# xiph/vorbis

Hardware: AMD Instinct MI355X
Metric: audio blocks/s (2048-sample MDCT+psy) @1/2/4/8 GPU; % HBM roofline (higher is better)
Workload: dtype f32

## Files before the change

include/vorbis_amd.h:

```cpp
#ifndef VORBIS_AMD_H
#define VORBIS_AMD_H

#include <stddef.h>
#include <stdint.h>
#include "vamd_setup.h"

#ifdef __cplusplus
extern "C" {
#endif

#define VAMD_OK        0
#define VAMD_EFAULT   (-129)
#define VAMD_EIMPL    (-130)
#define VAMD_EINVAL   (-131)
#define VAMD_EVERSION (-134)
#define VAMD_EDOMAIN    (-140)
#define VAMD_ENONFINITE (-141)

#define VAMD_BLOCKTYPE_IMPULSE    0
#define VAMD_BLOCKTYPE_PADDING    1
#define VAMD_BLOCKTYPE_TRANSITION 0
#define VAMD_BLOCKTYPE_LONG       1

#define VAMD_POSTS_STRIDE 32
// ... 5 lines not shown
#define vamd_create(ctx, setup_blob, blob_bytes, device) \
  vamd_create_abi((ctx), (setup_blob), (blob_bytes), (device), VAMD_ABI_VERSION)

void vamd_destroy(vamd_ctx *ctx);

const char *vamd_last_error(const vamd_ctx *ctx);

int vamd_set_stream(vamd_ctx *ctx, void *hip_stream);

int vamd_reserve(vamd_ctx *ctx, int W, long max_blocks);

int vamd_profile(vamd_ctx *ctx, int enable);
int vamd_stage_ms(vamd_ctx *ctx, float *ms, int nstages, int *runs);

int vamd_debug_cycles(vamd_ctx *ctx, int enable, unsigned long long *out80);

int vamd_clock_probe(vamd_ctx *ctx, unsigned long long *acc3);

int vamd_calib_copy(vamd_ctx *ctx, void *dst, const void *src, size_t bytes);

int vamd_channels(const vamd_ctx *ctx);
int vamd_blocksize(const vamd_ctx *ctx, int W);
int vamd_posts(const vamd_ctx *ctx, int W);


int vamd_mdct_forward_batch(vamd_ctx *ctx, int W, const float *in, float *out, long nframes);

typedef struct vamd_batch_desc {
  int         W;
  long        nblocks;
// ... 263 lines not shown
```

vorbis_amd/api.py:

```python
import ctypes as C
import os
import struct

import numpy as np

_HERE = os.path.dirname(os.path.abspath(__file__))

VAMD_OK, VAMD_EFAULT, VAMD_EIMPL, VAMD_EINVAL, VAMD_EVERSION, VAMD_EDOMAIN, VAMD_ENONFINITE = 0, -129, -130, -131, -134, -140, -141
ABI_VERSION = 9
QUANT_LIMIT_SQUARE, QUANT_LIMIT_INT = 46340, 0x7fffff80
STATUS_RANGE, STATUS_NONFINITE = 1, 2
LEVEL_TRANSFORM, LEVEL_PSY, LEVEL_FULL = 1, 2, 3
POSTS_STRIDE = 32
BLOCKTYPE_IMPULSE, BLOCKTYPE_PADDING, BLOCKTYPE_TRANSITION, BLOCKTYPE_LONG = 0, 1, 0, 1

EXPORTED_SYMBOLS = ["vamd_create_abi", "vamd_encode_blocks", "vamd_clock_probe", "vamd_quant_limit", "vamd_config_string", "vamd_destroy", "vamd_last_error", "vamd_set_stream", "vamd_reserve",
                    "vamd_channels", "vamd_blocksize", "vamd_posts", "vamd_mdct_forward_batch",
                    "vamd_analyze_batch", "vamd_analyze_stream", "vamd_analyze_block", "vamd_profile",
                    "vamd_stage_ms", "vamd_debug_cycles", "vamd_analyze_stream_mixed", "vamd_envelope_search_batch",
                    "vamd_envelope_search", "vamd_envelope_geometry", "vamd_residue_capacity", "vamd_analyze_block_res", "vamd_analyze_batch_managed", "vamd_analyze_block_managed",
                    "vamd_packet_capacity", "vamd_encode_block", "vamd_submaps", "vamd_residue_offset", "vamd_analyze_streams_mixed",
                    "vamd_plan_streams", "vamd_gather_blocks", "vamd_plan_fetch",
                    "vamd_batcher_create", "vamd_batcher_destroy", "vamd_batcher_attach", "vamd_batcher_detach",
                    "vamd_batcher_encode_block", "vamd_batcher_last_error", "vamd_batcher_stats", "vamd_batcher_context", "vamd_batcher_report",
                    "vamd_input_status", "vamd_calib_copy", "vamd_abi_version", "vamd_plan_streams_whole", "vamd_plan_streams_whole_v", "vamd_feed_wrote_v", "vamd_device_count", "vamd_batcher_create_multi",
                    "vamd_feed_create", "vamd_feed_destroy", "vamd_feed_lanes", "vamd_feed_device", "vamd_feed_buffer", "vamd_feed_wrote",
                    "vamd_feed_packets", "vamd_feed_release", "vamd_feed_last_error", "vamd_feed_create_live", "vamd_feed_wrote_live",
                    "vamd_analyze_streams_mixed_managed", "vamd_bitrate_init_states", "vamd_bitrate_walk",
                    "vamd_feed_ogg_headers", "vamd_feed_ogg_serials", "vamd_feed_ogg", "vamd_feed_ogg_headers_live",
                    "vamd_feed_ogg_comments", "vamd_feed_ogg_flush",
                    "vamd_feed_buffer_on", "vamd_feed_wrote_device", "vamd_feed_wrote_live_device", "vamd_feed_source_done",
                    "vamd_analyze_batch_synth", "vamd_synth_streams", "vamd_synth_check", "vamd_feed_decoded"]
PACKETBLOBS = 15

# ... 124 lines not shown
    L.vamd_destroy.restype = None
    L.vamd_last_error.argtypes = [_vp]
    L.vamd_last_error.restype = C.c_char_p
    L.vamd_set_stream.argtypes = [_vp, _vp]
    L.vamd_input_status.argtypes = [_vp, C.POINTER(C.c_long), C.POINTER(C.c_long)]
    L.vamd_reserve.argtypes = [_vp, C.c_int, C.c_long]
    L.vamd_channels.argtypes = [_vp]
    L.vamd_blocksize.argtypes = [_vp, C.c_int]
    L.vamd_posts.argtypes = [_vp, C.c_int]
    L.vamd_mdct_forward_batch.argtypes = [_vp, C.c_int, _vp, _vp, C.c_long]
    L.vamd_analyze_batch.argtypes = [_vp, C.POINTER(_Desc), C.POINTER(_IO), C.c_int]
    L.vamd_analyze_stream.argtypes = [_vp, C.POINTER(_Desc), C.POINTER(_IO), C.POINTER(C.c_float)]
    L.vamd_analyze_block.argtypes = [_vp, C.POINTER(_vp), C.c_int, C.c_int, C.c_int, C.c_int, C.c_float, _vp, _vp,
                                     _vp, _vp, _vp, _vp, C.POINTER(C.c_float)]
    L.vamd_debug_cycles.argtypes = [_vp, C.c_int, _vp]
    L.vamd_calib_copy.argtypes = [_vp, _vp, _vp, C.c_size_t]
    L.vamd_analyze_stream_mixed.argtypes = [_vp, C.POINTER(_Desc), C.POINTER(_IO), C.POINTER(_Desc), C.POINTER(_IO), _vp,
                                            C.c_long, C.POINTER(C.c_float)]
    L.vamd_analyze_streams_mixed.argtypes = [_vp, C.POINTER(_Desc), C.POINTER(_IO), C.POINTER(_Desc), C.POINTER(_IO), _vp, _vp,
                                             C.c_long, C.c_long, _vp]
    L.vamd_envelope_search_batch.argtypes = [_vp, _vp, C.c_long, C.c_long, C.c_long, C.c_long, _vp, _vp]
    L.vamd_envelope_search.argtypes = [_vp, C.POINTER(_vp), C.c_long, _vp, _vp]
    L.vamd_envelope_geometry.argtypes = [_vp, C.POINTER(C.c_int), C.POINTER(C.c_int)]
    L.vamd_residue_capacity.argtypes = [_vp, C.c_int]
    L.vamd_analyze_block_res.argtypes = [_vp, C.POINTER(_vp), C.c_int, C.c_int, C.c_int, C.c_int, C.c_float] + [_vp] * 10
    L.vamd_analyze_batch_managed.argtypes = [_vp, C.POINTER(_Desc), C.POINTER(_IO), C.POINTER(_MIO)]
    L.vamd_analyze_batch_synth.argtypes = [_vp, C.POINTER(_Desc), C.POINTER(_IO), _vp]
    L.vamd_synth_check.argtypes = [_vp, C.c_int]
    L.vamd_synth_streams.argtypes = [_vp, C.POINTER(_Plan), C.c_long, C.c_long, _vp, _vp, _vp, _vp, _vp]
    L.vamd_analyze_block_managed.argtypes = [_vp, C.POINTER(_vp), C.c_int, C.c_int, C.c_int, C.c_int, C.c_float] + [_vp] * 9
# ... 122 lines not shown
        runs = C.c_int(0)
        self._check(self.L.vamd_stage_ms(self.h, ms, 8, C.byref(runs)))
        return dict(zip(self.STAGES, [float(x) for x in ms])), runs.value

    def clock_probe(self, acc):
        if acc is not None:
            self._need_tensor(acc, self.torch.int64, "acc", numel=3)
        self._clk = acc
        self._check(self.L.vamd_clock_probe(self.h, _vp(acc.data_ptr()) if acc is not None else None))

    def debug_cycles(self, enable=True, read=False):
        out = np.zeros(80, dtype=np.uint64)
        self._check(self.L.vamd_debug_cycles(self.h, 1 if enable else 0, _vp(out.ctypes.data) if read else None))
        return out.reshape(5, 16)

    def calib_copy(self, dst, src):
        nbytes = src.numel() * src.element_size()
        assert dst.numel() * dst.element_size() == nbytes
        self._check(self.L.vamd_calib_copy(self.h, _vp(dst.data_ptr()), _vp(src.data_ptr()), nbytes))

    def reserve(self, W, max_blocks):
        self._check(self.L.vamd_reserve(self.h, W, max_blocks))

    def input_status(self):
        a, b = C.c_long(0), C.c_long(0)
        r = self.L.vamd_input_status(self.h, C.byref(a), C.byref(b))
        if r not in (VAMD_OK, VAMD_EDOMAIN, VAMD_ENONFINITE):
            self._check(r)
        self.last_input_code = r
        return int(a.value), int(b.value)
# ... 1076 lines not shown
```

vorbis_amd/csrc/k_tone.h:

```cpp
#pragma once
#include "vamd_wave.h"
#include "vamd_params.h"

namespace vamd {

#define VAMD_NEGINF (-9999.f)
#define VAMD_LINES_PAD(nl) (((nl) + 31) & ~31)

VAMD_HOSTDEV int seed_pad_lo(int linesper) { return (VAMD_EHMER_OFFSET * linesper + (linesper >> 1) + 3) & ~3; }
VAMD_HOSTDEV int seed_pad_hi(int linesper) { return ((VAMD_EHMER_MAX - VAMD_EHMER_OFFSET) * linesper + 3) & ~3; }
template <int LP = 0>
VAMD_DEV void seed_curve_scatter(float *seed, const float *__restrict__ band_rows ,
                                 int stride, float amp, int oc, int linesper_rt, float dBoffset, bool active) {
  const int linesper = LP ? LP : linesper_rt;
  int choice = (int)(((double)(amp + dBoffset) - 30.) * (double).1f);
  choice = choice < 0 ? 0 : choice;
  choice = choice > VAMD_P_LEVELS - 1 ? VAMD_P_LEVELS - 1 : choice;
  const F4 *__restrict__ row = (const F4 *)(band_rows + choice * stride);
  float *p = seed + (oc - VAMD_EHMER_OFFSET * linesper - (linesper >> 1));
  int p0 = VAMD_EHMER_MAX, p1 = 0;
  if (active) {
    const F2 posts = *(const F2 *)((const float *)row + VAMD_EHMER_MAX);
    p0 = (int)posts.x;
    p1 = (int)posts.y;
// ... 18 lines not shown
#define VAMD_TF_RUN_LINES 8
#endif
#ifndef VAMD_TF_GROUP_FOLD
#define VAMD_TF_GROUP_FOLD 0
#endif
#if VAMD_GPU
VAMD_DEV float tone_min(float a, float b) { return __builtin_amdgcn_fmed3f(a, b, VAMD_NEGINF); }
#define VAMD_TF_RUN_LOOP _Pragma("unroll 1")
#else
VAMD_DEV float tone_min(float a, float b) { return b < a ? b : a; }
#define VAMD_TF_RUN_LOOP
#endif
#include "k_tone_fold.inc"

#define VAMD_RING 16
VAMD_DEV int tone_chase_thread(const float *__restrict__ seeds, int linesper, int n, float *ring_amp, int *ring_pos,
                               int rstride, int rlane, unsigned short *__restrict__ surv) {
  int stack = 0, hmax = 0;
  unsigned long long wlo = 0, whi = 0;
  int nw = 0;
  auto emit = [&](int pos) {
    wlo = (wlo >> 16) | (whi << 48);
    whi = (whi >> 16) | ((unsigned long long)(unsigned)pos << 48);
    nw++;
    if ((nw & 7) == 0) {
      unsigned long long *dst = (unsigned long long *)(surv + nw - 8);
      dst[0] = wlo;
      dst[1] = whi;
    }
  };
  float a1 = 0.f, a2 = 0.f;
  int p1 = 0, p2 = 0;
  const F4 *q = (const F4 *)seeds;
  const int nblk = (n + 31) >> 5;
  F4 w[8];
#pragma unroll
  for (int k = 0; k < 8; k++) w[k] = q[k];
  for (int b = 0; b < nblk; b++) {
    float blk[32];
#pragma unroll
    for (int k = 0; k < 8; k++) blk[4 * k] = w[k].x, blk[4 * k + 1] = w[k].y, blk[4 * k + 2] = w[k].z, blk[4 * k + 3] = w[k].w;
    if (b + 1 < nblk) {
#pragma unroll
      for (int k = 0; k < 8; k++) w[k] = q[8 * b + 8 + k];
    }
#pragma unroll
    for (int j = 0; j < 32; j++) {
      const int i = (b << 5) + j;
      if (i < n) {
        const float s = blk[j];
        if (stack >= 2) {
          while (!(s < a1) && i < p1 + linesper && a1 <= a2 && i < p2 + linesper) {
            stack--;
            a1 = a2;
            p1 = p2;
            if (stack < 2) break;
            const int slot = (stack - 2) & (VAMD_RING - 1);
            a2 = ring_amp[slot * rstride + rlane];
            p2 = ring_pos[slot * rstride + rlane];
          }
        }
        const int slot = stack & (VAMD_RING - 1);
        if (stack == hmax) {
          if (stack >= VAMD_RING) emit(ring_pos[slot * rstride + rlane]);
          hmax++;
        }
        ring_amp[slot * rstride + rlane] = s;
        ring_pos[slot * rstride + rlane] = i;
        stack++;
        a2 = a1;
        p2 = p1;
        a1 = s;
        p1 = i;
      }
    }
  }
  for (int k = hmax > VAMD_RING ? hmax - VAMD_RING : 0; k < stack; k++) emit(ring_pos[(k & (VAMD_RING - 1)) * rstride + rlane]);
  for (int k = nw & ~7; k < nw; k++) {
    const int sh = 16 * (8 - (nw & 7) + (k & 7));
    surv[k] = (unsigned short)(sh < 64 ? wlo >> sh : whi >> (sh - 64));
  }
  return stack;
}

struct ChaseChunk {
  uint32_t popped;
  uint32_t sig_in;
  uint32_t sig_out;
  int exact;
};
VAMD_DEV ChaseChunk chase_chunk(const float *seeds, int linesper, int n, int s, int e, int warm, uint32_t enter,
                                float *ring_amp, int *ring_pos, int rstride, int rlane) {
  ChaseChunk out;
  out.popped = out.sig_in = out.sig_out = 0;
  const int ws = warm < 0 ? s : (s - warm > 0 ? s - warm : 0);
  out.exact = ws == 0;
  const int stop = e + linesper - 1 < n ? e + linesper - 1 : n;
  int stack = 0;
  float a1 = 0.f, a2 = 0.f;
  int p1 = 0, p2 = 0;
  if (warm < 0 && s > 0) {
    auto push = [&](float a, int pos) {
      const int slot = stack & (VAMD_RING - 1);
      ring_amp[slot * rstride + rlane] = a;
      ring_pos[slot * rstride + rlane] = pos;
      stack++;
      a2 = a1;
      p2 = p1;
      a1 = a;
      p1 = pos;
    };
    push(0.f, -(1 << 24));
    const int lo = s - linesper + 1;
    for (int k = 0; k < linesper - 1; k++)
      if (lo + k >= 0 && ((enter >> k) & 1u)) push(seeds[lo + k], lo + k);
  }
  auto window = [&](int t) {
    uint32_t m = 0;
    const int lo = t - linesper + 1;
    for (int k = stack - 1; k >= 0 && k >= stack - linesper; k--) {
      const int pos = k == stack - 1 ? p1 : (k == stack - 2 ? p2 : ring_pos[(k & (VAMD_RING - 1)) * rstride + rlane]);
      if (pos < lo) break;
      m |= 1u << (pos - lo);
    }
    return m;
  };
  for (int i = ws; i < stop; i++) {
    if (i == s) out.sig_in = window(s);
    if (i == e) out.sig_out = window(e);
    const float sv = seeds[i];
    if (stack >= 2) {
      while (!(sv < a1) && i < p1 + linesper && a1 <= a2 && i < p2 + linesper) {
        if (p1 >= s && p1 < e) out.popped |= 1u << (p1 - s);
        stack--;
        a1 = a2;
        p1 = p2;
        if (stack < 2) break;
        const int slot = (stack - 2) & (VAMD_RING - 1);
        a2 = ring_amp[slot * rstride + rlane];
        p2 = ring_pos[slot * rstride + rlane];
      }
    }
    const int slot = stack & (VAMD_RING - 1);
    ring_amp[slot * rstride + rlane] = sv;
    ring_pos[slot * rstride + rlane] = i;
    stack++;
    a2 = a1;
    p2 = p1;
    a1 = sv;
    p1 = i;
  }
  return out;
}

template <int LP>
VAMD_DEV ChaseChunk chase_chunk_regs(const float *seeds, int n, int s, int e, int cs, int warm, uint32_t enter) {
  constexpr int WN = LP - 1;
  constexpr uint32_t WMASK = (1u << WN) - 1u;
  ChaseChunk out;
  out.popped = out.sig_in = out.sig_out = 0;
  const int ws = warm < 0 ? s : s - warm;
  out.exact = ws <= 0;
  const int stop = e + LP - 1 < n ? e + LP - 1 : n;
  const int steps = (warm < 0 ? 0 : warm) + cs + LP - 1;
  uint32_t m = 0;
  float st[WN];
#pragma unroll
// ... 177 lines not shown
```

vorbis_amd/csrc/vamd_batch.h:

```cpp
#pragma once
struct WsPlan {
  float *mdct_raw, *logmdct, *logfft, *noise, *tone, *mdct, *local, *ampin, *ampglob, *seed;
  float *peaks;
  unsigned short *surv;
  int32_t *nsurv;
  ilog_t *ilogmask;
  int32_t *iwork, *posts, *post_valid, *nonzero;
  int32_t *wrapped;
  unsigned char *status;
};

static int run_peaks_stride(const PsyP &P) { return (P.nruns + 3) & ~3; }

static int plan(vamd_ctx *c, int W, long nb, const vamd_batch_io *io, int level, WsPlan *p) {
  const size_t ch = c->B.channels, n2 = c->B.bs[W] / 2;
  const size_t per = (size_t)nb * ch * n2 * 4;
  p->wrapped = nullptr;
  void *v;
#define PICK(field, user, slot, bytes)                     \
  do {                                                     \
    if (user) {                                            \
      p->field = user;                                     \
    } else {                                               \
      int r__ = ws_get(c, W, vamd_ctx::slot, (bytes), &v); \
// ... 26 lines not shown
    PICK(iwork, io ? io->iwork : nullptr, WS_IWORK, per);
    PICK(posts, io ? io->posts : nullptr, WS_POSTS, (size_t)nb * ch * VAMD_POSTS_STRIDE * 4);
    PICK(post_valid, io ? io->post_valid : nullptr, WS_POSTVALID, (size_t)nb * ch * 4);
    PICK(nonzero, io ? io->nonzero : nullptr, WS_NONZERO, (size_t)nb * ch * 4);
    if (io && io->packets) PICK(wrapped, (int32_t *)nullptr, WS_WRAPPED, (size_t)nb * ch * VAMD_POSTS_STRIDE * 4);
  }
#undef PICK
  return VAMD_OK;
}

int vamd_reserve(vamd_ctx *c, int W, long max_blocks) {
  DeviceGuard dev_guard(c);
  if (!c || (W != 0 && W != 1) || max_blocks < 1) return VAMD_EINVAL;
  WsPlan p;
  return plan(c, W, max_blocks, nullptr, VAMD_LEVEL_FULL, &p);
}

#define VAMD_SWITCH_LOGN(logn)   \
  switch (logn) {                \
    case 8: VAMD_GO(8); break;   \
    case 9: VAMD_GO(9); break;   \
    case 10: VAMD_GO(10); break; \
    case 11: VAMD_GO(11); break; \
    case 12: VAMD_GO(12); break; \
    default: VAMD_GO(0);         \
  }
#define VAMD_SWITCH_BINS(n2)                                                                \
  switch (n2) {                                                                             \
    case 32: VAMD_GO(5); break;                                                             \
    case 64: VAMD_GO(6); break;                                                             \
// ... 272 lines not shown
  return ((size_t)(nlp + (P0.ngroups > P1.ngroups ? P0.ngroups : P1.ngroups) + 1) * 4 + 15) & ~(size_t)15;
}
static bool fold_in_floor(const vamd_ctx *c, const BatchRun *R, int level) {
  const bool fold_env = !c->K.fold_separate;
  return fold_env && level >= VAMD_LEVEL_FULL && !R->M && c->B.xf[R->W].n / 2 <= 64 * 4 * VAMD_QPL;
}

static long noise_teams_per_cu(const vamd_ctx *c, int n2, size_t lds, bool overlap, bool alone, bool fold_later) {
  const int nw = n2 >= 256 ? 4 : (n2 >= 64 ? n2 / 64 : 1);
  long per_cu = (long)(c->lds_per_block / lds);
  if (per_cu > 32 / nw) per_cu = 32 / nw;
  const int noise_cap = c->K.noise_teams;
  if (noise_cap > 0) {
    if (per_cu > noise_cap) per_cu = noise_cap;
  } else if (overlap) {
    const int beside = c->K.noise_waves > 0 ? c->K.noise_waves : (alone ? 20 : 24);
    const long cap = (fold_later ? beside : 16) / nw;
    if (per_cu > cap) per_cu = cap > 0 ? cap : 1;
  }
  return per_cu < 1 ? 1 : per_cu;
}

static void launch_masks(vamd_ctx *c, BatchRun *R, int level, bool forked, bool alone) {
  if (R->nb == 0 || level < VAMD_LEVEL_PSY) return;
  const int W = R->W, ch = c->B.channels;
  const WsPlan &p = R->p;
  const DescP &d = R->d;
  const PsyP &P0 = c->B.psy[2 * W], &P1 = c->B.psy[2 * W + 1];
  const int n2 = c->B.xf[W].n / 2, nl = P0.total_octave_lines;
  const unsigned gcb = (unsigned)(R->nb * ch);
  hipStream_t s = c->stream;
  const bool overlap = masks_overlap(c, R);
  const bool fold_later = fold_in_floor(c, R, level);
  if (overlap && !forked) {
    (void)hipEventRecord(c->ev_fork, c->stream);
    (void)hipStreamWaitEvent(c->side, c->ev_fork, 0);
  }
  const int nlp = VAMD_LINES_PAD(nl);
  const size_t seed_lds = (size_t)(seed_pad_lo(P0.eighth_octave_lines) + nlp + seed_pad_hi(P0.eighth_octave_lines)) * 4;
  const long wave_max_cb = c->K.chase_wave_max;
  const bool by_wave = (long)gcb <= wave_max_cb && P0.eighth_octave_lines <= 16 && nl <= 2048;
  const bool lp8 = P0.eighth_octave_lines == 8 && P1.eighth_octave_lines == 8;
  const bool merge_env = !c->K.masks_separate;
  const bool merged = merge_env && !overlap && by_wave && lp8;
  if (merged) {
    const size_t nlds = (size_t)5 * VAMD_NZ_STRIDE(n2) * 4, tlds = seed_lds + (size_t)VAMD_RING * 8;
#define VAMD_GO(L)                                                                                                          \
  hipLaunchKernelGGL((k_noise_tone<L, 8>), dim3(2 * gcb), dim3(64 * NoiseGeom<L>::NW), nlds > tlds ? nlds : tlds, s, P0, P1, d, ch, \
                     (long)gcb, p.mdct_raw, p.noise, nlp, run_peaks_stride(P0), p.peaks, p.local, p.ampglob,                  \
                     R->make_ampmax ? p.ampglob : nullptr, p.seed, p.surv, p.nsurv)
    VAMD_SWITCH_BINS(n2)
#undef VAMD_GO
    prof_mark(c, VAMD_ST_NOISE);
  } else {
    const size_t lds = (size_t)5 * VAMD_NZ_STRIDE(n2) * 4;
    const long per_cu = noise_teams_per_cu(c, n2, lds, overlap, alone, fold_later);
    const unsigned grid = (unsigned)((long)gcb < per_cu * c->num_cus ? (long)gcb : per_cu * c->num_cus);
#define VAMD_GO(L)                                                                                                    \
  hipLaunchKernelGGL(k_noise<L>, dim3(grid), dim3(64 * NoiseGeom<L>::NW), lds, s, P0, P1, d, ch, (long)gcb, p.mdct_raw, \
                     p.noise)
    VAMD_SWITCH_BINS(n2)
#undef VAMD_GO
    prof_mark(c, VAMD_ST_NOISE);
  }
  if (overlap) s = c->side;
  {
    if (merged) {
    } else if (by_wave && lp8) {
      hipLaunchKernelGGL(k_tone_seed_chase<8>, dim3(gcb), dim3(64), seed_lds + (size_t)VAMD_RING * 8, s, P0, P1, d, ch, nlp,
                         run_peaks_stride(P0), p.peaks, p.local, p.ampglob, R->make_ampmax ? p.ampglob : nullptr, p.seed, p.surv,
                         p.nsurv);
    } else {
      if (lp8)
        hipLaunchKernelGGL(k_tone_seed<8>, dim3(gcb), dim3(64), seed_lds, s, P0, P1, d, ch, nlp, run_peaks_stride(P0), p.peaks, p.local,
                           p.ampglob, R->make_ampmax ? p.ampglob : nullptr, p.seed);
      else
        hipLaunchKernelGGL(k_tone_seed<0>, dim3(gcb), dim3(64), seed_lds, s, P0, P1, d, ch, nlp, run_peaks_stride(P0), p.peaks, p.local,
                           p.ampglob, R->make_ampmax ? p.ampglob : nullptr, p.seed);
      if (by_wave)
        hipLaunchKernelGGL(k_tone_chase_wave, dim3(gcb), dim3(64), (size_t)nlp * 4 + (size_t)VAMD_RING * 64 * 8, s,
                           P0.eighth_octave_lines, nl, nlp, d, p.seed, p.surv, p.nsurv);
      else
        hipLaunchKernelGGL(k_tone_chase, dim3((gcb + VAMD_CHASE_LANES - 1) / VAMD_CHASE_LANES), dim3(VAMD_CHASE_LANES),
                           (size_t)VAMD_RING * VAMD_CHASE_LANES * 8, s,
                           P0.eighth_octave_lines, nl, nlp, (long)gcb, d, p.seed, p.surv, p.nsurv);
    }
    if (!fold_later)
      hipLaunchKernelGGL(k_tone_fold, dim3(gcb), dim3(64), fold_lds_bytes(nlp, P0, P1), s, P0, P1, d, ch, nlp, p.seed, p.surv,
                         p.nsurv, p.local, p.tone);
  }
  if (overlap) (void)hipEventRecord(join_event(c, R), c->side);
}

static void launch_floor_on(vamd_ctx *c, BatchRun *R, int level) {
  if (R->nb == 0) return;
  const ResBufs &rb = R->rb;
  const int W = R->W, ch = c->B.channels;
  const WsPlan &p = R->p;
  const DescP &d = R->d;
  const vamd_managed_io *M = R->M;
// ... 351 lines not shown
```

vorbis_amd/csrc/vamd_kernels.h:

```cpp
#pragma once
extern __shared__ __attribute__((aligned(16))) unsigned char vamd_smem[];

__device__ __forceinline__ int d_lW(const DescP &d, long b) { return d.lW ? d.lW[b] : d.u_lW; }
__device__ __forceinline__ int d_nW(const DescP &d, long b) { return d.nW ? d.nW[b] : d.u_nW; }
__device__ __forceinline__ int d_bt(const DescP &d, long b) { return d.blocktype ? d.blocktype[b] : d.u_blocktype; }
__device__ __forceinline__ float d_amp(const DescP &d, long b) { return d.ampmax_in ? d.ampmax_in[b] : d.u_ampmax_in; }
__device__ __forceinline__ void flag_range(const DescP &d, long i) {
  const unsigned char old = d.status[i];
  if (!(old & VAMD_STATUS_RANGE)) {
    d.status[i] = old | VAMD_STATUS_RANGE;
    if (!old) atomicAdd(d.bad, 1u);
  }
}

#define VAMD_XF_WAVES 8
#ifndef VAMD_FLOOR_PAIR_MIN_LONG
#define VAMD_FLOOR_PAIR_MIN_LONG 0x7fffffffL
#endif
#ifndef VAMD_FLOOR_PAIR_MIN_SHORT
#define VAMD_FLOOR_PAIR_MIN_SHORT 16384L
#endif

struct XformLds {
  XformP P;
// ... 394 lines not shown
  const PsyP &P = d_bt(d, blk) ? P1 : P0;
  float g_amp;
  if (ampmax_make) {
    g_amp = d_amp(d, blk);
    for (int c = 0; c < ch; c++) {
      const float l = local_ampmax[blk * ch + c];
      if (l > g_amp) g_amp = l;
    }
    if (LANE == 0 && cb == blk * ch) ampmax_make[blk] = g_amp;
  } else {
    g_amp = ampmax_glob[blk];
  }
  const int nl = P.total_octave_lines;
  float *seed = (float *)vamd_smem + seed_pad_lo(LP);
  float *ring_amp = seed + nlp + seed_pad_hi(LP);
  int *ring_pos = (int *)(ring_amp + VAMD_RING);
  PhaseClock pc;
  pc.start(d.dbg ? d.dbg + 32 : nullptr);
  tone_seed_block<LP>(P, peaks + cb * nrp, g_amp, local_ampmax[cb], seed, pc);
  WAVE_FOR(i, nlp) {
    if (i >= nl) seed[i] = VAMD_NEGINF;
    seed_g[cb * nlp + i] = seed[i];
  }
  WAVE_SYNC();
  const int cs = (nl + 63) / 64;
  const int s0 = LANE * cs < nl ? LANE * cs : nl, e0 = s0 + cs < nl ? s0 + cs : nl;
  unsigned short *out = surv + cb * nlp;
  bool accepted = false;
  ChaseChunk r;
  r.popped = r.sig_in = r.sig_out = 0;
  r.exact = 1;
// ... 15 lines not shown
        const ChaseChunk t = chase_chunk_regs<LP>(seed, nl, s0, e0, cs, -1, prev_out);
        used = prev_out;
        r.popped = t.popped;
        r.sig_out = t.sig_out;
      }
    }
  }
  if (accepted) {
    const uint32_t alive = ~r.popped & (e0 - s0 >= 32 ? ~0u : ((1u << (e0 - s0)) - 1u));
    const int cnt = __builtin_popcount(alive);
    const int incl = wave_scan_sum(cnt);
    int at = incl - cnt;
    for (uint32_t m = alive; m; m &= m - 1) out[at++] = (unsigned short)(s0 + __builtin_ctz(m));
    if (LANE == 63) nsurv[cb] = incl;
  } else if (LANE == 0) {
    nsurv[cb] = tone_chase_thread(seed, LP, nl, ring_amp, ring_pos, 1, 0, out);
  }
  pc.mark(2);
  pc.flush();
}
template <int LP>
__global__ __launch_bounds__(64) void k_tone_seed_chase(PsyP P0, PsyP P1, DescP d, int ch, int nlp, int nrp,
                                                        const float *__restrict__ peaks,
                                                        const float *__restrict__ local_ampmax,
                                                        const float *__restrict__ ampmax_glob, float *__restrict__ ampmax_make,
                                                        float *__restrict__ seed_g, unsigned short *__restrict__ surv,
                                                        int *__restrict__ nsurv) {
  tone_seed_chase_run<LP>(P0, P1, d, ch, nlp, nrp, peaks, local_ampmax, ampmax_glob, ampmax_make, seed_g, surv, nsurv, blockIdx.x);
}

template <int LOGN2, int LP>
// ... 1 lines not shown
                                                                          const float *__restrict__ mdct_raw, float *__restrict__ noise,
                                                                          int nlp, int nrp, const float *__restrict__ peaks,
                                                                          const float *__restrict__ local_ampmax,
                                                                          const float *__restrict__ ampmax_glob, float *__restrict__ ampmax_make,
                                                                          float *__restrict__ seed_g, unsigned short *__restrict__ surv,
                                                                          int *__restrict__ nsurv) {
  if ((long)blockIdx.x < ncb) {
    noise_teams_once<LOGN2>(P0, P1, d, ch, mdct_raw, noise);
  } else if (threadIdx.x < 64) {
    tone_seed_chase_run<LP>(P0, P1, d, ch, nlp, nrp, peaks, local_ampmax, ampmax_glob, ampmax_make, seed_g, surv, nsurv,
                            (long)blockIdx.x - ncb);
  }
}

#define VAMD_CHASE_LANES 64
__global__ __launch_bounds__(64) void k_tone_chase(int linesper, int nl, int nlp, long ncb, DescP d,
                                                   const float *__restrict__ seed_g,
                                                   unsigned short *__restrict__ surv, int *__restrict__ nsurv) {
  float *ring_amp = (float *)vamd_smem;
  int *ring_pos = (int *)(ring_amp + VAMD_RING * VAMD_CHASE_LANES);
  const long cb = (long)blockIdx.x * VAMD_CHASE_LANES + threadIdx.x;
  PhaseClock pc;
  pc.start(d.dbg ? d.dbg + 32 : nullptr);
  const bool probe = d.clk && blockIdx.x == 0 && threadIdx.x == 0;
  unsigned long long w0 = 0;
  long long t0 = 0;
  if (probe) w0 = wall_clock64(), t0 = clock64();
  if (cb < ncb)
    nsurv[cb] = tone_chase_thread(seed_g + cb * nlp, linesper, nl, ring_amp, ring_pos, VAMD_CHASE_LANES, threadIdx.x, surv + cb * nlp);
  if (probe) {
    atomicAdd(d.clk, (unsigned long long)(clock64() - t0));
    atomicAdd(d.clk + 1, wall_clock64() - w0);
    atomicAdd(d.clk + 2, 1ull);
  }
  pc.mark(2);
  pc.flush();
}

__global__ __launch_bounds__(64) void k_tone_chase_wave(int linesper, int nl, int nlp, DescP d,
                                                        const float *__restrict__ seed_g,
                                                        unsigned short *__restrict__ surv, int *__restrict__ nsurv) {
  float *seed = (float *)vamd_smem;
  float *ring_amp = seed + nlp;
  int *ring_pos = (int *)(ring_amp + VAMD_RING * 64);
  const long cb = blockIdx.x;
  WAVE_FOR(q, nlp >> 2)((F4 *)seed)[q] = ((const F4 *)(seed_g + cb * nlp))[q];
  WAVE_SYNC();
  const int cs = (nl + 63) / 64;
  const int s0 = LANE * cs < nl ? LANE * cs : nl, e0 = s0 + cs < nl ? s0 + cs : nl;
  unsigned short *out = surv + cb * nlp;
  bool accepted = false;
  ChaseChunk r;
  r.popped = r.sig_in = r.sig_out = 0;
  r.exact = 1;
  unsigned long long fm = __ballot(s0 < nl && chase_flat_chunk(seed, s0, e0));
  int longest = 0;
  for (; fm && longest <= VAMD_CHASE_FLAT_MAX; longest++) fm &= fm << 1;
  if (longest <= VAMD_CHASE_FLAT_MAX) {
    if (s0 < nl) r = chase_chunk(seed, linesper, nl, s0, e0, VAMD_CHASE_WARM * linesper, 0, ring_amp, ring_pos, 64, LANE);
    uint32_t used = r.sig_in;
    for (int rd = 0; rd <= VAMD_CHASE_ROUNDS; rd++) {
      const uint32_t prev_out = (uint32_t)wave_shift_up1((int)r.sig_out, 0);
      const bool need = s0 < nl && !r.exact && used != prev_out;
      if (!__any(need)) {
        accepted = true;
        break;
      }
      if (rd == VAMD_CHASE_ROUNDS) break;
      if (need) {
        const ChaseChunk t = chase_chunk(seed, linesper, nl, s0, e0, -1, prev_out, ring_amp, ring_pos, 64, LANE);
        used = prev_out;
        r.popped = t.popped;
        r.sig_out = t.sig_out;
      }
    }
  }
  if (accepted) {
    const uint32_t alive = ~r.popped & (e0 - s0 >= 32 ? ~0u : ((1u << (e0 - s0)) - 1u));
    const int cnt = __builtin_popcount(alive);
    const int incl = wave_scan_sum(cnt);
    int at = incl - cnt;
    for (uint32_t m = alive; m; m &= m - 1) out[at++] = (unsigned short)(s0 + __builtin_ctz(m));
    if (LANE == 63) nsurv[cb] = incl;
  } else if (LANE == 0) {
    nsurv[cb] = tone_chase_thread(seed, linesper, nl, ring_amp, ring_pos, 64, 0, out);
  }
}

__global__ __launch_bounds__(64) void k_tone_fold(PsyP P0, PsyP P1, DescP d, int ch, int nlp,
                                                  const float *__restrict__ seed_g,
                                                  const unsigned short *__restrict__ surv,
                                                  const int *__restrict__ nsurv,
                                                  const float *__restrict__ local_ampmax, float *__restrict__ tone) {
  const long cb = blockIdx.x;
  const long blk = cb / ch;
  const PsyP &P = d_bt(d, blk) ? P1 : P0;
  const int n2 = P.n;
  float *seed = (float *)vamd_smem;
  float *gmin = seed + nlp;
  PhaseClock pc;
// ... 877 lines not shown
```

vorbis_amd/csrc/vamd_knobs.h:

```cpp
#pragma once
#include <stdio.h>
#include <stdlib.h>
#include <string.h>

namespace vamd {

struct Knobs {
  bool verbose = false;
  int batch_lanes = 8;
  int batch_eager = -1;
  int batch_join = -1;
  long batch_spin_below = -1;
  bool test = false;
  bool no_overlap = false;
  bool couple_band_set = false;
  int couple_band_log2 = 0;
  int xf_waves_cap = 0;
  long res_team_max = 2048;
  bool res_in_lds = false;
  long pack_pair_max = 2048;
  bool pack_per_packet = false;
  bool fold_separate = false;
  long chase_wave_max = 32768;
  bool masks_separate = false;
  int noise_teams = 0;
  int noise_waves = 0;
  long floor_lds_pad = 0;
  long floor_pair_min = -1;
  int floor_pair_w = 3;
  bool stage_copies = false;
  bool env_untiled = false;
  int xf_variant = -1;
  long fail_envelope_after = -1;
  long fail_encode_after = -1;
  long feed_slice = 2048;
  long feed_out_bytes = 0;
  long plan_window = 0;
};

inline Knobs read_knobs() {
  {
    Knobs k;
// ... 10 lines not shown
      k.no_overlap = on("VAMD_NO_OVERLAP");
      k.couple_band_set = on("VAMD_COUPLE_BAND_LOG2");
      k.couple_band_log2 = (int)num("VAMD_COUPLE_BAND_LOG2", 0);
      k.xf_waves_cap = (int)num("VAMD_XF_WAVES_CAP", 0);
      k.res_team_max = num("VAMD_RES_TEAM_MAX", k.res_team_max);
      k.res_in_lds = on("VAMD_RES_IN_LDS");
      k.pack_pair_max = num("VAMD_PACK_PAIR_MAX", k.pack_pair_max);
      k.pack_per_packet = on("VAMD_PACK_PER_PACKET");
      k.fold_separate = on("VAMD_FOLD_SEPARATE");
      k.chase_wave_max = num("VAMD_CHASE_WAVE_MAX", k.chase_wave_max);
      k.masks_separate = on("VAMD_MASKS_SEPARATE");
      k.noise_teams = (int)num("VAMD_NOISE_TEAMS", 0);
      k.noise_waves = (int)num("VAMD_NOISE_WAVES", k.noise_waves);
      if (k.noise_waves < 4 || k.noise_waves > 32) k.noise_waves = 0;
      k.floor_lds_pad = num("VAMD_FLOOR_LDS_PAD", 0);
      k.floor_pair_min = num("VAMD_FLOOR_PAIR_MIN", -1);
      k.floor_pair_w = (int)num("VAMD_FLOOR_PAIR_W", 3);
      k.stage_copies = on("VAMD_STAGE_COPIES");
      k.env_untiled = on("VAMD_ENV_UNTILED");
      k.xf_variant = (int)num("VAMD_XF_VARIANT", -1);
      k.fail_envelope_after = num("VAMD_FAIL_ENVELOPE_AFTER", -1);
      k.fail_encode_after = num("VAMD_FAIL_ENCODE_AFTER", -1);
      k.feed_slice = num("VAMD_FEED_SLICE", k.feed_slice);
      k.feed_out_bytes = num("VAMD_FEED_OUT_BYTES", 0);
      k.plan_window = num("VAMD_PLAN_WINDOW", 0);
    }
    return k;
  }
}

inline void knobs_string(const Knobs &k, char *buf, size_t cap) {
  int n = snprintf(buf, cap, "VAMD_VERBOSE=%d VAMD_BATCH_LANES=%d VAMD_BATCH_EAGER=%d VAMD_BATCH_JOIN=%d VAMD_BATCH_SPIN_BELOW=%ld VAMD_TEST_KNOBS=%d",
                   (int)k.verbose, k.batch_lanes, k.batch_eager, k.batch_join, k.batch_spin_below, (int)k.test);
  if (k.test && n > 0 && (size_t)n < cap)
    snprintf(buf + n, cap - (size_t)n,
             " VAMD_NO_OVERLAP=%d VAMD_COUPLE_BAND_LOG2=%s%d VAMD_XF_WAVES_CAP=%d VAMD_RES_TEAM_MAX=%ld VAMD_RES_IN_LDS=%d VAMD_PACK_PAIR_MAX=%ld VAMD_PACK_PER_PACKET=%d"
             " VAMD_FOLD_SEPARATE=%d VAMD_CHASE_WAVE_MAX=%ld VAMD_MASKS_SEPARATE=%d VAMD_NOISE_TEAMS=%d VAMD_NOISE_WAVES=%d VAMD_FLOOR_LDS_PAD=%ld"
             " VAMD_FLOOR_PAIR_MIN=%ld VAMD_FLOOR_PAIR_W=%d VAMD_STAGE_COPIES=%d VAMD_ENV_UNTILED=%d VAMD_XF_VARIANT=%d VAMD_FAIL_ENVELOPE_AFTER=%ld"
             " VAMD_FAIL_ENCODE_AFTER=%ld VAMD_FEED_SLICE=%ld VAMD_FEED_OUT_BYTES=%ld VAMD_PLAN_WINDOW=%ld",
             (int)k.no_overlap, k.couple_band_set ? "" : "unset:", k.couple_band_log2, k.xf_waves_cap, k.res_team_max, (int)k.res_in_lds,
             k.pack_pair_max, (int)k.pack_per_packet, (int)k.fold_separate, k.chase_wave_max, (int)k.masks_separate, k.noise_teams, k.noise_waves, k.floor_lds_pad,
             k.floor_pair_min, k.floor_pair_w, (int)k.stage_copies, (int)k.env_untiled, k.xf_variant, k.fail_envelope_after,
             k.fail_encode_after, k.feed_slice, k.feed_out_bytes, k.plan_window);
}

}
```

Baseline: 20.89 million.

## Shrink tone-chase LDS ring to 8 slots when eighth-octave lines fit

```diff
diff --git a/include/vorbis_amd.h b/include/vorbis_amd.h
--- a/include/vorbis_amd.h
+++ b/include/vorbis_amd.h
@@ -43,6 +43,9 @@
 int vamd_stage_ms(vamd_ctx *ctx, float *ms, int nstages, int *runs);
 
 int vamd_debug_cycles(vamd_ctx *ctx, int enable, unsigned long long *out80);
+
+int vamd_debug_survivors(vamd_ctx *ctx, int W, long channel_blocks, float *seed, uint16_t *surv, int32_t *nsurv,
+                         int32_t *row_lines, int32_t *lines);
 
 int vamd_clock_probe(vamd_ctx *ctx, unsigned long long *acc3);
 
diff --git a/vorbis_amd/api.py b/vorbis_amd/api.py
--- a/vorbis_amd/api.py
+++ b/vorbis_amd/api.py
@@ -17,7 +17,7 @@
 EXPORTED_SYMBOLS = ["vamd_create_abi", "vamd_encode_blocks", "vamd_clock_probe", "vamd_quant_limit", "vamd_config_string", "vamd_destroy", "vamd_last_error", "vamd_set_stream", "vamd_reserve",
                     "vamd_channels", "vamd_blocksize", "vamd_posts", "vamd_mdct_forward_batch",
                     "vamd_analyze_batch", "vamd_analyze_stream", "vamd_analyze_block", "vamd_profile",
-                    "vamd_stage_ms", "vamd_debug_cycles", "vamd_analyze_stream_mixed", "vamd_envelope_search_batch",
+                    "vamd_stage_ms", "vamd_debug_cycles", "vamd_debug_survivors", "vamd_analyze_stream_mixed", "vamd_envelope_search_batch",
                     "vamd_envelope_search", "vamd_envelope_geometry", "vamd_residue_capacity", "vamd_analyze_block_res", "vamd_analyze_batch_managed", "vamd_analyze_block_managed",
                     "vamd_packet_capacity", "vamd_encode_block", "vamd_submaps", "vamd_residue_offset", "vamd_analyze_streams_mixed",
                     "vamd_plan_streams", "vamd_gather_blocks", "vamd_plan_fetch",
@@ -172,6 +172,7 @@
     L.vamd_analyze_block.argtypes = [_vp, C.POINTER(_vp), C.c_int, C.c_int, C.c_int, C.c_int, C.c_float, _vp, _vp,
                                      _vp, _vp, _vp, _vp, C.POINTER(C.c_float)]
     L.vamd_debug_cycles.argtypes = [_vp, C.c_int, _vp]
+    L.vamd_debug_survivors.argtypes = [_vp, C.c_int, C.c_long, _vp, _vp, _vp, C.POINTER(C.c_int32), C.POINTER(C.c_int32)]
     L.vamd_calib_copy.argtypes = [_vp, _vp, _vp, C.c_size_t]
     L.vamd_analyze_stream_mixed.argtypes = [_vp, C.POINTER(_Desc), C.POINTER(_IO), C.POINTER(_Desc), C.POINTER(_IO), _vp,
                                             C.c_long, C.POINTER(C.c_float)]
@@ -324,6 +325,16 @@
         self._check(self.L.vamd_debug_cycles(self.h, 1 if enable else 0, _vp(out.ctypes.data) if read else None))
         return out.reshape(5, 16)
 
+    def debug_survivors(self, W, channel_blocks):
+        row, nl = C.c_int32(), C.c_int32()
+        self._check(self.L.vamd_debug_survivors(self.h, W, 0, None, None, None, C.byref(row), C.byref(nl)))
+        seed = np.zeros((channel_blocks, row.value), np.float32)
+        surv = np.zeros((channel_blocks, row.value), np.uint16)
+        nsurv = np.zeros(channel_blocks, np.int32)
+        self._check(self.L.vamd_debug_survivors(self.h, W, channel_blocks, _vp(seed.ctypes.data), _vp(surv.ctypes.data),
+                                                _vp(nsurv.ctypes.data), None, None))
+        return seed, surv, nsurv, nl.value
+
     def calib_copy(self, dst, src):
         nbytes = src.numel() * src.element_size()
         assert dst.numel() * dst.element_size() == nbytes
diff --git a/vorbis_amd/csrc/k_tone.h b/vorbis_amd/csrc/k_tone.h
--- a/vorbis_amd/csrc/k_tone.h
+++ b/vorbis_amd/csrc/k_tone.h
@@ -56,8 +56,20 @@
 #include "k_tone_fold.inc"
 
 #define VAMD_RING 16
-VAMD_DEV int tone_chase_thread(const float *__restrict__ seeds, int linesper, int n, float *ring_amp, int *ring_pos,
-                               int rstride, int rlane, unsigned short *__restrict__ surv) {
+#ifndef VAMD_CHASE_RING
+#define VAMD_CHASE_RING 8
+#endif
+#ifndef VAMD_CHASE_GUARD
+#define VAMD_CHASE_GUARD 0
+#endif
+#ifndef VAMD_CHASE_PREFETCH
+#define VAMD_CHASE_PREFETCH 0
+#endif
+static_assert(VAMD_CHASE_RING == 8 || VAMD_CHASE_RING == VAMD_RING, "VAMD_CHASE_RING is 8 or 16");
+constexpr int chase_ring_slots(int linesper) { return linesper <= 8 ? VAMD_CHASE_RING : VAMD_RING; }
+template <int RING>
+VAMD_DEV int tone_chase_ring(const float *__restrict__ seeds, int linesper, int n, float *ring_amp, int *ring_pos,
+                             int rstride, int rlane, unsigned short *__restrict__ surv) {
   int stack = 0, hmax = 0;
   unsigned long long wlo = 0, whi = 0;
   int nw = 0;
@@ -76,16 +88,24 @@
   const F4 *q = (const F4 *)seeds;
   const int nblk = (n + 31) >> 5;
   F4 w[8];
+#if VAMD_CHASE_PREFETCH
 #pragma unroll
   for (int k = 0; k < 8; k++) w[k] = q[k];
+#endif
   for (int b = 0; b < nblk; b++) {
     float blk[32];
+#if !VAMD_CHASE_PREFETCH
+#pragma unroll
+    for (int k = 0; k < 8; k++) w[k] = q[8 * b + k];
+#endif
 #pragma unroll
     for (int k = 0; k < 8; k++) blk[4 * k] = w[k].x, blk[4 * k + 1] = w[k].y, blk[4 * k + 2] = w[k].z, blk[4 * k + 3] = w[k].w;
+#if VAMD_CHASE_PREFETCH
     if (b + 1 < nblk) {
 #pragma unroll
       for (int k = 0; k < 8; k++) w[k] = q[8 * b + 8 + k];
     }
+#endif
 #pragma unroll
     for (int j = 0; j < 32; j++) {
       const int i = (b << 5) + j;
@@ -97,14 +117,20 @@
             a1 = a2;
             p1 = p2;
             if (stack < 2) break;
-            const int slot = (stack - 2) & (VAMD_RING - 1);
+            const int slot = (stack - 2) & (RING - 1);
             a2 = ring_amp[slot * rstride + rlane];
             p2 = ring_pos[slot * rstride + rlane];
+#if VAMD_CHASE_GUARD
+            if (hmax > stack - 2 + RING) {
+              VAMD_CHASE_GUARD_HIT();
+              p2 = -(1 << 24);
+            }
+#endif
           }
         }
-        const int slot = stack & (VAMD_RING - 1);
+        const int slot = stack & (RING - 1);
         if (stack == hmax) {
-          if (stack >= VAMD_RING) emit(ring_pos[slot * rstride + rlane]);
+          if (stack >= RING) emit(ring_pos[slot * rstride + rlane]);
           hmax++;
         }
         ring_amp[slot * rstride + rlane] = s;
@@ -117,12 +143,17 @@
       }
     }
   }
-  for (int k = hmax > VAMD_RING ? hmax - VAMD_RING : 0; k < stack; k++) emit(ring_pos[(k & (VAMD_RING - 1)) * rstride + rlane]);
+  for (int k = hmax > RING ? hmax - RING : 0; k < stack; k++) emit(ring_pos[(k & (RING - 1)) * rstride + rlane]);
   for (int k = nw & ~7; k < nw; k++) {
     const int sh = 16 * (8 - (nw & 7) + (k & 7));
     surv[k] = (unsigned short)(sh < 64 ? wlo >> sh : whi >> (sh - 64));
   }
   return stack;
+}
+VAMD_DEV int tone_chase_thread(const float *__restrict__ seeds, int linesper, int n, float *ring_amp, int *ring_pos,
+                               int rstride, int rlane, unsigned short *__restrict__ surv) {
+  if (chase_ring_slots(linesper) == VAMD_CHASE_RING) return tone_chase_ring<VAMD_CHASE_RING>(seeds, linesper, n, ring_amp, ring_pos, rstride, rlane, surv);
+  return tone_chase_ring<VAMD_RING>(seeds, linesper, n, ring_amp, ring_pos, rstride, rlane, surv);
 }
 
 struct ChaseChunk {
@@ -131,8 +162,9 @@
   uint32_t sig_out;
   int exact;
 };
-VAMD_DEV ChaseChunk chase_chunk(const float *seeds, int linesper, int n, int s, int e, int warm, uint32_t enter,
-                                float *ring_amp, int *ring_pos, int rstride, int rlane) {
+template <int RING>
+VAMD_DEV ChaseChunk chase_chunk_ring(const float *seeds, int linesper, int n, int s, int e, int warm, uint32_t enter,
+                                     float *ring_amp, int *ring_pos, int rstride, int rlane) {
   ChaseChunk out;
   out.popped = out.sig_in = out.sig_out = 0;
   const int ws = warm < 0 ? s : (s - warm > 0 ? s - warm : 0);
@@ -143,7 +175,7 @@
   int p1 = 0, p2 = 0;
   if (warm < 0 && s > 0) {
     auto push = [&](float a, int pos) {
-      const int slot = stack & (VAMD_RING - 1);
+      const int slot = stack & (RING - 1);
       ring_amp[slot * rstride + rlane] = a;
       ring_pos[slot * rstride + rlane] = pos;
       stack++;
@@ -161,7 +193,7 @@
     uint32_t m = 0;
     const int lo = t - linesper + 1;
     for (int k = stack - 1; k >= 0 && k >= stack - linesper; k--) {
-      const int pos = k == stack - 1 ? p1 : (k == stack - 2 ? p2 : ring_pos[(k & (VAMD_RING - 1)) * rstride + rlane]);
+      const int pos = k == stack - 1 ? p1 : (k == stack - 2 ? p2 : ring_pos[(k & (RING - 1)) * rstride + rlane]);
       if (pos < lo) break;
       m |= 1u << (pos - lo);
     }
@@ -178,12 +210,12 @@
         a1 = a2;
         p1 = p2;
         if (stack < 2) break;
-        const int slot = (stack - 2) & (VAMD_RING - 1);
+        const int slot = (stack - 2) & (RING - 1);
         a2 = ring_amp[slot * rstride + rlane];
         p2 = ring_pos[slot * rstride + rlane];
       }
     }
-    const int slot = stack & (VAMD_RING - 1);
+    const int slot = stack & (RING - 1);
     ring_amp[slot * rstride + rlane] = sv;
     ring_pos[slot * rstride + rlane] = i;
     stack++;
@@ -193,6 +225,11 @@
     p1 = i;
   }
   return out;
+}
+VAMD_DEV ChaseChunk chase_chunk(const float *seeds, int linesper, int n, int s, int e, int warm, uint32_t enter,
+                                float *ring_amp, int *ring_pos, int rstride, int rlane) {
+  if (chase_ring_slots(linesper) == VAMD_CHASE_RING) return chase_chunk_ring<VAMD_CHASE_RING>(seeds, linesper, n, s, e, warm, enter, ring_amp, ring_pos, rstride, rlane);
+  return chase_chunk_ring<VAMD_RING>(seeds, linesper, n, s, e, warm, enter, ring_amp, ring_pos, rstride, rlane);
 }
 
 template <int LP>
diff --git a/vorbis_amd/csrc/vamd_batch.h b/vorbis_amd/csrc/vamd_batch.h
--- a/vorbis_amd/csrc/vamd_batch.h
+++ b/vorbis_amd/csrc/vamd_batch.h
@@ -64,6 +64,24 @@
   if (!c || (W != 0 && W != 1) || max_blocks < 1) return VAMD_EINVAL;
   WsPlan p;
   return plan(c, W, max_blocks, nullptr, VAMD_LEVEL_FULL, &p);
+}
+
+int vamd_debug_survivors(vamd_ctx *c, int W, long ncb, float *seed, uint16_t *surv, int32_t *nsurv, int32_t *row_lines,
+                         int32_t *lines) {
+  DeviceGuard dev_guard(c);
+  if (!c || (W != 0 && W != 1) || ncb < 0) return VAMD_EINVAL;
+  const size_t nl = (size_t)c->B.psy[2 * W].total_octave_lines, nlp = (size_t)VAMD_LINES_PAD(nl);
+  if (row_lines) *row_lines = (int32_t)nlp;
+  if (lines) *lines = (int32_t)nl;
+  if (!seed && !surv && !nsurv) return VAMD_OK;
+  const DevBuf &bs = c->ws[W][vamd_ctx::WS_SEED], &bv = c->ws[W][vamd_ctx::WS_SURV], &bn = c->ws[W][vamd_ctx::WS_NSURV];
+  if (bs.bytes < (size_t)ncb * nlp * 4 || bv.bytes < (size_t)ncb * nlp * 2 || bn.bytes < (size_t)ncb * 4)
+    return fail(c, VAMD_EINVAL, "no batch of that size has left survivor lists");
+  HIP_TRY(c, hipStreamSynchronize(c->stream));
+  if (seed) HIP_TRY(c, hipMemcpy(seed, bs.p, (size_t)ncb * nlp * 4, hipMemcpyDeviceToHost));
+  if (surv) HIP_TRY(c, hipMemcpy(surv, bv.p, (size_t)ncb * nlp * 2, hipMemcpyDeviceToHost));
+  if (nsurv) HIP_TRY(c, hipMemcpy(nsurv, bn.p, (size_t)ncb * 4, hipMemcpyDeviceToHost));
+  return VAMD_OK;
 }
 
 #define VAMD_SWITCH_LOGN(logn)   \
@@ -366,7 +384,7 @@
   if (noise_cap > 0) {
     if (per_cu > noise_cap) per_cu = noise_cap;
   } else if (overlap) {
-    const int beside = c->K.noise_waves > 0 ? c->K.noise_waves : (alone ? 20 : 24);
+    const int beside = c->K.noise_waves > 0 ? c->K.noise_waves : (alone && n2 < 1024 ? 20 : 24);
     const long cap = (fold_later ? beside : 16) / nw;
     if (per_cu > cap) per_cu = cap > 0 ? cap : 1;
   }
@@ -393,10 +411,12 @@
   const long wave_max_cb = c->K.chase_wave_max;
   const bool by_wave = (long)gcb <= wave_max_cb && P0.eighth_octave_lines <= 16 && nl <= 2048;
   const bool lp8 = P0.eighth_octave_lines == 8 && P1.eighth_octave_lines == 8;
+  const bool ring8 = P0.eighth_octave_lines <= 8 && P1.eighth_octave_lines <= 8 && VAMD_CHASE_RING < VAMD_RING;
+  const size_t ring_slots = ring8 ? VAMD_CHASE_RING : VAMD_RING;
   const bool merge_env = !c->K.masks_separate;
   const bool merged = merge_env && !overlap && by_wave && lp8;
   if (merged) {
-    const size_t nlds = (size_t)5 * VAMD_NZ_STRIDE(n2) * 4, tlds = seed_lds + (size_t)VAMD_RING * 8;
+    const size_t nlds = (size_t)5 * VAMD_NZ_STRIDE(n2) * 4, tlds = seed_lds + (size_t)chase_ring_slots(8) * 8;
 #define VAMD_GO(L)                                                                                                          \
   hipLaunchKernelGGL((k_noise_tone<L, 8>), dim3(2 * gcb), dim3(64 * NoiseGeom<L>::NW), nlds > tlds ? nlds : tlds, s, P0, P1, d, ch, \
                      (long)gcb, p.mdct_raw, p.noise, nlp, run_peaks_stride(P0), p.peaks, p.local, p.ampglob,                  \
@@ -419,7 +439,7 @@
   {
     if (merged) {
     } else if (by_wave && lp8) {
-      hipLaunchKernelGGL(k_tone_seed_chase<8>, dim3(gcb), dim3(64), seed_lds + (size_t)VAMD_RING * 8, s, P0, P1, d, ch, nlp,
+      hipLaunchKernelGGL(k_tone_seed_chase<8>, dim3(gcb), dim3(64), seed_lds + (size_t)chase_ring_slots(8) * 8, s, P0, P1, d, ch, nlp,
                          run_peaks_stride(P0), p.peaks, p.local, p.ampglob, R->make_ampmax ? p.ampglob : nullptr, p.seed, p.surv,
                          p.nsurv);
     } else {
@@ -429,13 +449,21 @@
       else
         hipLaunchKernelGGL(k_tone_seed<0>, dim3(gcb), dim3(64), seed_lds, s, P0, P1, d, ch, nlp, run_peaks_stride(P0), p.peaks, p.local,
                            p.ampglob, R->make_ampmax ? p.ampglob : nullptr, p.seed);
-      if (by_wave)
-        hipLaunchKernelGGL(k_tone_chase_wave, dim3(gcb), dim3(64), (size_t)nlp * 4 + (size_t)VAMD_RING * 64 * 8, s,
-                           P0.eighth_octave_lines, nl, nlp, d, p.seed, p.surv, p.nsurv);
-      else
-        hipLaunchKernelGGL(k_tone_chase, dim3((gcb + VAMD_CHASE_LANES - 1) / VAMD_CHASE_LANES), dim3(VAMD_CHASE_LANES),
-                           (size_t)VAMD_RING * VAMD_CHASE_LANES * 8, s,
-                           P0.eighth_octave_lines, nl, nlp, (long)gcb, d, p.seed, p.surv, p.nsurv);
+      const size_t chase_pad = (size_t)c->K.chase_lds_pad;
+#define VAMD_GO(RING)                                                                                                          \
+  if (by_wave)                                                                                                                 \
+    hipLaunchKernelGGL(k_tone_chase_wave<RING>, dim3(gcb), dim3(64), (size_t)nlp * 4 + (size_t)RING * 64 * 8, s,               \
+                       P0.eighth_octave_lines, nl, nlp, d, p.seed, p.surv, p.nsurv);                                           \
+  else                                                                                                                         \
+    hipLaunchKernelGGL(k_tone_chase<RING>, dim3((gcb + VAMD_CHASE_LANES - 1) / VAMD_CHASE_LANES), dim3(VAMD_CHASE_LANES),      \
+                       (size_t)RING * VAMD_CHASE_LANES * 8 + chase_pad, s, P0.eighth_octave_lines, nl, nlp, (long)gcb, d, p.seed, \
+                       p.surv, p.nsurv)
+      if (ring_slots == VAMD_RING) {
+        VAMD_GO(VAMD_RING);
+      } else {
+        VAMD_GO(VAMD_CHASE_RING);
+      }
+#undef VAMD_GO
     }
     if (!fold_later)
       hipLaunchKernelGGL(k_tone_fold, dim3(gcb), dim3(64), fold_lds_bytes(nlp, P0, P1), s, P0, P1, d, ch, nlp, p.seed, p.surv,
diff --git a/vorbis_amd/csrc/vamd_kernels.h b/vorbis_amd/csrc/vamd_kernels.h
--- a/vorbis_amd/csrc/vamd_kernels.h
+++ b/vorbis_amd/csrc/vamd_kernels.h
@@ -432,7 +432,8 @@
   const int nl = P.total_octave_lines;
   float *seed = (float *)vamd_smem + seed_pad_lo(LP);
   float *ring_amp = seed + nlp + seed_pad_hi(LP);
-  int *ring_pos = (int *)(ring_amp + VAMD_RING);
+  constexpr int RING = chase_ring_slots(LP);
+  int *ring_pos = (int *)(ring_amp + RING);
   PhaseClock pc;
   pc.start(d.dbg ? d.dbg + 32 : nullptr);
   tone_seed_block<LP>(P, peaks + cb * nrp, g_amp, local_ampmax[cb], seed, pc);
@@ -478,7 +479,7 @@
     for (uint32_t m = alive; m; m &= m - 1) out[at++] = (unsigned short)(s0 + __builtin_ctz(m));
     if (LANE == 63) nsurv[cb] = incl;
   } else if (LANE == 0) {
-    nsurv[cb] = tone_chase_thread(seed, LP, nl, ring_amp, ring_pos, 1, 0, out);
+    nsurv[cb] = tone_chase_ring<RING>(seed, LP, nl, ring_amp, ring_pos, 1, 0, out);
   }
   pc.mark(2);
   pc.flush();
@@ -510,11 +511,12 @@
 }
 
 #define VAMD_CHASE_LANES 64
+template <int RING>
 __global__ __launch_bounds__(64) void k_tone_chase(int linesper, int nl, int nlp, long ncb, DescP d,
                                                    const float *__restrict__ seed_g,
                                                    unsigned short *__restrict__ surv, int *__restrict__ nsurv) {
   float *ring_amp = (float *)vamd_smem;
-  int *ring_pos = (int *)(ring_amp + VAMD_RING * VAMD_CHASE_LANES);
+  int *ring_pos = (int *)(ring_amp + RING * VAMD_CHASE_LANES);
   const long cb = (long)blockIdx.x * VAMD_CHASE_LANES + threadIdx.x;
   PhaseClock pc;
   pc.start(d.dbg ? d.dbg + 32 : nullptr);
@@ -523,7 +525,7 @@
   long long t0 = 0;
   if (probe) w0 = wall_clock64(), t0 = clock64();
   if (cb < ncb)
-    nsurv[cb] = tone_chase_thread(seed_g + cb * nlp, linesper, nl, ring_amp, ring_pos, VAMD_CHASE_LANES, threadIdx.x, surv + cb * nlp);
+    nsurv[cb] = tone_chase_ring<RING>(seed_g + cb * nlp, linesper, nl, ring_amp, ring_pos, VAMD_CHASE_LANES, threadIdx.x, surv + cb * nlp);
   if (probe) {
     atomicAdd(d.clk, (unsigned long long)(clock64() - t0));
     atomicAdd(d.clk + 1, wall_clock64() - w0);
@@ -533,12 +535,13 @@
   pc.flush();
 }
 
+template <int RING>
 __global__ __launch_bounds__(64) void k_tone_chase_wave(int linesper, int nl, int nlp, DescP d,
                                                         const float *__restrict__ seed_g,
                                                         unsigned short *__restrict__ surv, int *__restrict__ nsurv) {
   float *seed = (float *)vamd_smem;
   float *ring_amp = seed + nlp;
-  int *ring_pos = (int *)(ring_amp + VAMD_RING * 64);
+  int *ring_pos = (int *)(ring_amp + RING * 64);
   const long cb = blockIdx.x;
   WAVE_FOR(q, nlp >> 2)((F4 *)seed)[q] = ((const F4 *)(seed_g + cb * nlp))[q];
   WAVE_SYNC();
@@ -553,7 +556,7 @@
   int longest = 0;
   for (; fm && longest <= VAMD_CHASE_FLAT_MAX; longest++) fm &= fm << 1;
   if (longest <= VAMD_CHASE_FLAT_MAX) {
-    if (s0 < nl) r = chase_chunk(seed, linesper, nl, s0, e0, VAMD_CHASE_WARM * linesper, 0, ring_amp, ring_pos, 64, LANE);
+    if (s0 < nl) r = chase_chunk_ring<RING>(seed, linesper, nl, s0, e0, VAMD_CHASE_WARM * linesper, 0, ring_amp, ring_pos, 64, LANE);
     uint32_t used = r.sig_in;
     for (int rd = 0; rd <= VAMD_CHASE_ROUNDS; rd++) {
       const uint32_t prev_out = (uint32_t)wave_shift_up1((int)r.sig_out, 0);
@@ -564,7 +567,7 @@
       }
       if (rd == VAMD_CHASE_ROUNDS) break;
       if (need) {
-        const ChaseChunk t = chase_chunk(seed, linesper, nl, s0, e0, -1, prev_out, ring_amp, ring_pos, 64, LANE);
+        const ChaseChunk t = chase_chunk_ring<RING>(seed, linesper, nl, s0, e0, -1, prev_out, ring_amp, ring_pos, 64, LANE);
         used = prev_out;
         r.popped = t.popped;
         r.sig_out = t.sig_out;
@@ -579,7 +582,7 @@
     for (uint32_t m = alive; m; m &= m - 1) out[at++] = (unsigned short)(s0 + __builtin_ctz(m));
     if (LANE == 63) nsurv[cb] = incl;
   } else if (LANE == 0) {
-    nsurv[cb] = tone_chase_thread(seed, linesper, nl, ring_amp, ring_pos, 64, 0, out);
+    nsurv[cb] = tone_chase_ring<RING>(seed, linesper, nl, ring_amp, ring_pos, 64, 0, out);
   }
 }
 
diff --git a/vorbis_amd/csrc/vamd_knobs.h b/vorbis_amd/csrc/vamd_knobs.h
--- a/vorbis_amd/csrc/vamd_knobs.h
+++ b/vorbis_amd/csrc/vamd_knobs.h
@@ -26,6 +26,7 @@
   int noise_teams = 0;
   int noise_waves = 0;
   long floor_lds_pad = 0;
+  long chase_lds_pad = 0;
   long floor_pair_min = -1;
   int floor_pair_w = 3;
   bool stage_copies = false;
@@ -66,6 +67,8 @@
       k.noise_waves = (int)num("VAMD_NOISE_WAVES", k.noise_waves);
       if (k.noise_waves < 4 || k.noise_waves > 32) k.noise_waves = 0;
       k.floor_lds_pad = num("VAMD_FLOOR_LDS_PAD", 0);
+      k.chase_lds_pad = num("VAMD_CHASE_LDS_PAD", 0);
+      if (k.chase_lds_pad < 0 || k.chase_lds_pad > 32768) k.chase_lds_pad = 0;
       k.floor_pair_min = num("VAMD_FLOOR_PAIR_MIN", -1);
       k.floor_pair_w = (int)num("VAMD_FLOOR_PAIR_W", 3);
       k.stage_copies = on("VAMD_STAGE_COPIES");
@@ -89,11 +92,11 @@
              " VAMD_NO_OVERLAP=%d VAMD_COUPLE_BAND_LOG2=%s%d VAMD_XF_WAVES_CAP=%d VAMD_RES_TEAM_MAX=%ld VAMD_RES_IN_LDS=%d VAMD_PACK_PAIR_MAX=%ld VAMD_PACK_PER_PACKET=%d"
              " VAMD_FOLD_SEPARATE=%d VAMD_CHASE_WAVE_MAX=%ld VAMD_MASKS_SEPARATE=%d VAMD_NOISE_TEAMS=%d VAMD_NOISE_WAVES=%d VAMD_FLOOR_LDS_PAD=%ld"
              " VAMD_FLOOR_PAIR_MIN=%ld VAMD_FLOOR_PAIR_W=%d VAMD_STAGE_COPIES=%d VAMD_ENV_UNTILED=%d VAMD_XF_VARIANT=%d VAMD_FAIL_ENVELOPE_AFTER=%ld"
-             " VAMD_FAIL_ENCODE_AFTER=%ld VAMD_FEED_SLICE=%ld VAMD_FEED_OUT_BYTES=%ld VAMD_PLAN_WINDOW=%ld",
+             " VAMD_FAIL_ENCODE_AFTER=%ld VAMD_FEED_SLICE=%ld VAMD_FEED_OUT_BYTES=%ld VAMD_PLAN_WINDOW=%ld VAMD_CHASE_LDS_PAD=%ld",
              (int)k.no_overlap, k.couple_band_set ? "" : "unset:", k.couple_band_log2, k.xf_waves_cap, k.res_team_max, (int)k.res_in_lds,
              k.pack_pair_max, (int)k.pack_per_packet, (int)k.fold_separate, k.chase_wave_max, (int)k.masks_separate, k.noise_teams, k.noise_waves, k.floor_lds_pad,
              k.floor_pair_min, k.floor_pair_w, (int)k.stage_copies, (int)k.env_untiled, k.xf_variant, k.fail_envelope_after,
-             k.fail_encode_after, k.feed_slice, k.feed_out_bytes, k.plan_window);
+             k.fail_encode_after, k.feed_slice, k.feed_out_bytes, k.plan_window, k.chase_lds_pad);
 }
 
 }
```

Measured after the change: 21.17 million (median of 6 runs). 1.4% higher.
